# manikya7022/Continual-Learning-for-Dynamic-Video-Quality-Enhancement

Measured on AMD Instinct MI355X. Metric: train frames/sec (2x SR, T=3, 540p->1080p), higher is better.
Workload: dtype bf16

## Files before the change

continual-learning-for-dynamic-video-quality-enhancement_amd/csrc/conv_common.h:

```cpp
#pragma once
#include "common.h"

namespace nvq {

constexpr int TH = 8;
constexpr int TW = 32;
constexpr int NVQ_SMALL_IMAGE_TILES = 32;
constexpr int WG_C = 32;
constexpr int WGRAD_MAX_WG = 512;
constexpr int WGRAD_MAX_SLABS = 1536;

static inline int choose_nt(int cout) { return cout <= 16 ? 16 : (cout <= 32 ? 32 : 64); }

#ifdef NVQ_DEBUG_TOOLS
void set_conv_debug_mode(int m);
#endif
void conv_occupancy_bf16(int* out);

typedef short s16x4 __attribute__((ext_vector_type(4)));
typedef unsigned u32x4 __attribute__((ext_vector_type(4)));

constexpr int KCB = 32;

__host__ __device__ constexpr int ws_stride_halfs(int taps, int NT) { return ((taps * 4 * NT * 8 + 2047) / 2048) * 2048; }
// ... 15 lines not shown
              float* wpack, hipStream_t s);
struct PackJobDev { const float* w; float* wp; int cout_w, cin_w, taps, transpose, cout_keep, NT, ncz, nkc; long total; };
constexpr int PACK_BATCH = 48;
struct PackJobTable { PackJobDev j[PACK_BATCH]; };
int pack_batch_bf16(const PackJobTable& t, int n, hipStream_t s);
PackJobDev pack_job_bf16(const nvq_pack_job& j);
int conv_forward_bf16(const nvq_conv_desc& d, int vec_ok, hipStream_t s);
int conv_wgrad_bf16(const nvq_wgrad_desc& d, int nsplit, int nci, int nco, int tilesX, int tilesY, int ntiles,
                    hipStream_t s);
int upsampler_tail_bf16(const nvq_conv_desc& d, const float* frames, int T, int t_center, int Cimg, int s, float* out,
                        unsigned char* pass, hipStream_t st);
int rdb_tail_bf16(const nvq_conv_desc& d3, const nvq_conv_desc& dl, int vec3, int vecl, hipStream_t s);
int conv_forward_m32(const nvq_conv_desc& d, int variant, int dbg, hipStream_t s);
void conv_occupancy_m32(int* out);
bool wgrad_m32_takes(const nvq_wgrad_desc& d);
int conv_wgrad_m32(const nvq_wgrad_desc& d, hipStream_t s);

__device__ __forceinline__ void wgrad_bias_partial(const nvq_wgrad_desc& d, float4 bsum, float* lds, int nco, int cic,
                                                   int coc) {
    if (cic != 0 || d.dbias == nullptr) return;
    __syncthreads();
    st4(lds + 4 * threadIdx.x, bsum);
    __syncthreads();
    if (threadIdx.x < 32) {
        const int q = threadIdx.x >> 2, e = threadIdx.x & 3;
        float s = 0.f;
        for (int k = 0; k < 32; ++k) s += lds[4 * (8 * k + q) + e];
        float* bp = d.workspace + (size_t)WGRAD_MAX_SLABS * 9 * WG_C * WG_C;
        bp[((size_t)blockIdx.x * nco + coc) * WG_C + threadIdx.x] = s;
    }
}
// ... 180 lines not shown
```

continual-learning-for-dynamic-video-quality-enhancement_amd/csrc/conv_igemm.hip:

```cpp
#include "conv_common.h"

namespace nvq {

constexpr int KC = 16;
constexpr int XS_LD = 20;

__device__ __forceinline__ float pack_f32_elem(const float* __restrict__ w, int cout_w, int cin_w, int taps, int transpose,
                                               int cout_keep, int NT, int nkc, long idx) {
    long t = idx;
    const int j = t & 3; t >>= 2;
    const int n = t % NT; t /= NT;
    const int g = t & 3; t >>= 2;
    const int tap = t % taps; t /= taps;
    const int kc = t % nkc; t /= nkc;
    const int cz = (int)t;
    const int co = cz * NT + n;
    const int ch = kc * KC + 4 * g + j;
    float v = 0.f;
    if (!transpose) {
        if (co < cout_w && ch < cin_w) v = w[((long)co * cin_w + ch) * taps + tap];
    } else {
        if (co < cout_keep && ch < cout_w) v = w[((long)ch * cin_w + co) * taps + (taps - 1 - tap)];
    }
    return v;
// ... 676 lines not shown
            else if (gs == 2) NVQ_LAUNCH_CONV(2, KS, 2);             \
            else NVQ_LAUNCH_CONV(1, KS, 4);                          \
        }                                                            \
    } while (0)
    if (d.ksize == 3) NVQ_LAUNCH_CONV_KS(3);
    else NVQ_LAUNCH_CONV_KS(1);
#undef NVQ_LAUNCH_CONV_KS
#undef NVQ_LAUNCH_CONV
    return check_launch("conv_forward");
}

size_t nvq_wgrad_workspace_bytes(void) {
    return (size_t)WGRAD_MAX_SLABS * 9 * WG_C * WG_C * sizeof(float) + (size_t)512 * 256 * sizeof(float);
}

static int wgrad_partial(const nvq_wgrad_desc* dp, nvq_wgrad_reduce_job* job, void* stream) {
    const nvq_wgrad_desc d = *dp;
    NVQ_REQUIRE(d.math == NVQ_MATH_F32 || d.math == NVQ_MATH_BF16, "conv_wgrad: math mode %d", d.math);
    NVQ_REQUIRE(d.ksize == 1 || d.ksize == 3, "conv_wgrad: ksize %d", d.ksize);
    NVQ_REQUIRE(d.cin % 4 == 0 && d.x_ld % 4 == 0 && d.x_coff % 4 == 0 && aligned16(d.x),
                "conv_wgrad: x must be 16-byte addressable");
    NVQ_REQUIRE(d.dy_ld % 4 == 0 && d.dy_coff % 4 == 0 && aligned16(d.dy),
                "conv_wgrad: dy must be 16-byte addressable");
    NVQ_REQUIRE(d.cin_w > 0 && d.cin_w <= d.cin && d.cout > 0, "conv_wgrad: channels");
    NVQ_REQUIRE(!(d.x_bf16 | d.dy_bf16) || d.math == NVQ_MATH_BF16, "conv_wgrad: bf16 tensors need NVQ_MATH_BF16");
    NVQ_REQUIRE(!d.x_bf16 || (d.cin % 8 == 0 && d.x_ld % 8 == 0 && d.x_coff % 8 == 0), "conv_wgrad: bf16 x alignment");
    NVQ_REQUIRE(!d.dy_bf16 || (d.cout % 8 == 0 && d.dy_ld % 8 == 0 && d.dy_coff % 8 == 0), "conv_wgrad: bf16 dy alignment");
    NVQ_REQUIRE(d.math != NVQ_MATH_BF16 || d.dy_coff + ((d.cout + 3) & ~3) <= d.dy_ld,
                "conv_wgrad(bf16): the dy slice must be readable up to a multiple of 4 channels");
    NVQ_REQUIRE(d.workspace_bytes >= nvq_wgrad_workspace_bytes(), "conv_wgrad: workspace too small");
    NVQ_REQUIRE(!d.x_plane || (d.math == NVQ_MATH_BF16 && d.x_bf16 && d.x_coff == 0 && d.cin % 32 == 0 &&
                               (d.x_ld == 32 || d.x_ld == 64 || d.x_ld == 128) && d.x_ld <= d.cin &&
                               (size_t)d.x_plane == (size_t)d.n * d.h * d.w * 32),
                "conv_wgrad: a slice-planar x needs NVQ_MATH_BF16, bf16 storage, cin %% 32 == 0, x_coff 0, x_ld in {32, 64, 128} "
                "and x_plane = n*h*w*32");
    const int taps = d.ksize * d.ksize;
    const int nci = (d.cin_w + WG_C - 1) / WG_C, nco = (d.cout + WG_C - 1) / WG_C;
    const int tilesX = (d.w + TW - 1) / TW, tilesY = (d.h + TH - 1) / TH;
    const int ntiles = tilesX * tilesY * d.n;
    int nsplit = WGRAD_MAX_WG / (nci * nco);
    if (nsplit < 1) nsplit = 1;
    if (nsplit > ntiles) nsplit = ntiles;
    if (nsplit >= 8) nsplit &= ~7;
    NVQ_REQUIRE((size_t)nsplit * nci * nco * taps * WG_C * WG_C * sizeof(float) <= d.workspace_bytes,
                "conv_wgrad: %d x %d channel chunks exceed the workspace", nci, nco);
    hipStream_t s = (hipStream_t)stream;
    const dim3 grid(nsplit, nci, nco);
    int rc;
    if (d.math == NVQ_MATH_BF16) {
        const int used = conv_wgrad_bf16(d, nsplit, nci, nco, tilesX, tilesY, ntiles, s);
        if (used < 0) return used;
        rc = check_launch("conv_wgrad_bf16");
        if (used > 0) nsplit = used;
    } else {
        if (d.ksize == 3)
            hipLaunchKernelGGL((wgrad_f32_kernel<3>), grid, dim3(256), 0, s, d, tilesX, tilesY, ntiles, nci, nco);
        else
            hipLaunchKernelGGL((wgrad_f32_kernel<1>), grid, dim3(256), 0, s, d, tilesX, tilesY, ntiles, nci, nco);
        rc = check_launch("conv_wgrad");
    }
    if (rc) return rc;
    *job = nvq_wgrad_reduce_job{d.workspace, d.workspace + (size_t)WGRAD_MAX_SLABS * 9 * WG_C * WG_C, d.dw, d.dbias, nsplit, nci,
                                nco, taps, d.cout, d.cin_w, d.alpha, d.accumulate};
    return NVQ_OK;
}

int nvq_conv_wgrad(const nvq_wgrad_desc* dp, void* stream) {
    nvq_wgrad_reduce_job j;
    const int rc = wgrad_partial(dp, &j, stream);
    if (rc) return rc;
    return launch_wgrad_reduce_bias(j.part, j.nsplit, j.nci, j.nco, j.taps, j.cout, j.cin_w, j.alpha, j.accumulate, j.dw,
                                    j.bias_part, j.dbias, (hipStream_t)stream);
}

int nvq_conv_wgrad_partial(const nvq_wgrad_desc* dp, nvq_wgrad_reduce_job* job, void* stream) {
    NVQ_REQUIRE(job != nullptr, "conv_wgrad_partial: job");
    return wgrad_partial(dp, job, stream);
}

int nvq_wgrad_reduce_batch(const nvq_wgrad_reduce_job* jobs, int n, void* stream) {
    NVQ_REQUIRE(n >= 0 && (n == 0 || jobs != nullptr), "wgrad_reduce_batch: jobs");
    for (int i = 0; i < n; ++i)
        NVQ_REQUIRE(jobs[i].part && jobs[i].dw && jobs[i].nsplit > 0 && jobs[i].nci > 0 && jobs[i].nco > 0 &&
                        (jobs[i].taps == 1 || jobs[i].taps == 9) && (!jobs[i].dbias || jobs[i].bias_part),
                    "wgrad_reduce_batch: job %d is not one nvq_conv_wgrad_partial filled in", i);
    for (int i0 = 0; i0 < n; i0 += WR_MAX_JOBS) {
        const int m = n - i0 < WR_MAX_JOBS ? n - i0 : WR_MAX_JOBS;
        WgradReduceTable t;
        long need = 1;
        for (int i = 0; i < m; ++i) {
            t.j[i] = jobs[i0 + i];
            const long total = (long)t.j[i].nci * t.j[i].nco * t.j[i].taps * WG_C * WG_C;
// ... 21 lines not shown
```

continual-learning-for-dynamic-video-quality-enhancement_amd/csrc/wgrad_m32.hip:

```cpp
#include <type_traits>
#include "conv_common.h"

namespace nvq {

namespace {

typedef float f32x16 __attribute__((ext_vector_type(16)));
typedef s16x4 __attribute__((address_space(3))) * lds_s16x4_ptr;

constexpr int WM_TR = 4;
constexpr int WM_NTHR = 512;
constexpr int WM_HW = TW + 2, WM_HH = 2 + 2, WM_NPY = WM_HW * WM_HH;
constexpr int WM_YBYTES = WM_NPY * 64;
constexpr int WM_UPX = 2 * TW;
constexpr int WM_DYT = 384;

__device__ __forceinline__ void gload16(u32x4& dst, const void* p) {
    asm volatile("global_load_dwordx4 %0, %1, off" : "=&v"(dst) : "v"(p) : "memory");
}
__device__ __forceinline__ void gload16s(u32x4& dst, const void* sbase, unsigned voff) {
    asm volatile("global_load_dwordx4 %0, %1, %2" : "=&v"(dst) : "v"(voff), "s"(sbase) : "memory");
}
template <int N>
__device__ __forceinline__ void vm_wait() {
    asm volatile("s_waitcnt vmcnt(%0)" ::"n"(N) : "memory");
}
__device__ __forceinline__ void hold(u32x4& r) { asm volatile("" : "+v"(r)); }

template <int NCI>
struct WmCfg {
    static constexpr int CB = (NCI + 1) / 2;
    static constexpr int UBYTES = WM_UPX * NCI * 64;
    static constexpr int XPIECES = WM_UPX * NCI * 4;
    static constexpr int XPT = (XPIECES + WM_NTHR - 1) / WM_NTHR;
    static constexpr int LDS = 2 * UBYTES + 2 * WM_YBYTES;
};

// ... 240 lines not shown
#pragma unroll
            for (int e = 0; e < 8; ++e) scratch[8 * dt + e] = bsum[e];
        }
        __syncthreads();
        if (tid < 32) {
            const int piece = tid >> 3, e = tid & 7;
            float sum = 0.f;
            for (int k = piece; k < WM_DYT; k += 4) sum += scratch[8 * k + e];
            float* bp = d.workspace + (size_t)WGRAD_MAX_SLABS * 9 * WG_C * WG_C;
            bp[(size_t)blockIdx.x * WG_C + tid] = sum;
        }
    }
    (void)dyw;
}

template <int NCI, int NCO>
__global__ __launch_bounds__(WM_NTHR, 4) void wgrad1_m32_kernel(const nvq_wgrad_desc d, int tilesX, int tilesY, int ntiles) {
    constexpr int UBYTES = WM_UPX * NCI * 64, YB = WM_UPX * NCO * 64;
    constexpr int XPT = (WM_UPX * NCI * 4 + WM_NTHR - 1) / WM_NTHR;
    constexpr int YTHR = WM_UPX * NCO * 4;
    static_assert(NCI <= 8 && NCO <= 2 && 2 * (UBYTES + YB) <= 80 * 1024, "1x1 configuration");
    __shared__ __attribute__((aligned(1024))) unsigned char lds[2 * (UBYTES + YB)];
    constexpr int YOFF = 2 * UBYTES;

    const int tid = threadIdx.x;
    const int lane = tid & 63;
    const int wave = __builtin_amdgcn_readfirstlane(tid >> 6);
    const int H = d.h, W = d.w;
    const int G = gridDim.x;
    const int mytiles = ((int)blockIdx.x < ntiles) ? (ntiles - 1 - (int)blockIdx.x) / G + 1 : 0;
    const int U = 2 * mytiles;
    const __bf16* x16 = reinterpret_cast<const __bf16*>(d.x);
    const __bf16* dy16 = reinterpret_cast<const __bf16*>(d.dy);
    const int LU = d.x_plane ? d.x_ld >> 5 : NCI;

    const int xcol = (tid >> 2) & 31, xsub = tid & 3, xrow = (wave >> 1) & 1, xblk0 = wave >> 2;
    const unsigned v_lead = (unsigned)((xcol * d.x_ld + 8 * xsub) * 2), v_plane = (unsigned)((xcol * 32 + 8 * xsub) * 2);
    const int ypx = tid / (4 * NCO), yq = tid % (4 * NCO), yrow = NCO == 2 ? wave >> 2 : (wave >> 1) & 1, ycol = ypx & 31;
    const bool ythr = tid < YTHR;
    const unsigned v_y = (unsigned)((ycol * d.dy_ld + 8 * yq) * 2);
    struct Set { u32x4 x[XPT]; u32x4 y; bool xok, yok; };
    constexpr int S = XPT + 1;
    int c_n = 0, c_ty = 0, c_tx = 0, c_unit = 0;
    {
        int bt = xcd_tile((int)blockIdx.x, ntiles);
        c_tx = bt % tilesX; bt /= tilesX;
        c_ty = bt % tilesY;
        c_n = bt / tilesY;
    }
    const int c_step = G >> 3;
    auto load = [&](int u, Set& st) {
        if ((u >> 1) != (c_unit >> 1)) {
            if ((G & 7) == 0) {
                c_tx += c_step;
                while (c_tx >= tilesX) { c_tx -= tilesX; ++c_ty; }
                while (c_ty >= tilesY) { c_ty -= tilesY; ++c_n; }
            } else {
// ... 11 lines not shown
            st.xok = row_ok && xcol < W - x0;
            const unsigned vl = st.xok ? v_lead : 0u, vp = st.xok ? v_plane : 0u;
#pragma unroll
            for (int k = 0; k < XPT; ++k) {
                const int blk = xblk0 + 2 * k < NCI ? xblk0 + 2 * k : 0;
                if (blk < LU) gload16s(st.x[k], x16 + ((size_t)rel * (unsigned)d.x_ld + d.x_coff + 32u * blk), vl);
                else gload16s(st.x[k], x16 + ((size_t)blk * d.x_plane + rel * 32u), vp);
            }
        }
        {
            const bool row_ok = y0 + yrow < H;
            const size_t rel = (size_t)((c_n * H + (row_ok ? y0 + yrow : y0)) * W + x0);
            st.yok = ythr && row_ok && ycol < W - x0;
            gload16s(st.y, dy16 + (rel * d.dy_ld + d.dy_coff), st.yok ? v_y : 0u);
        }
    };
    float bsum[8];
#pragma unroll
    for (int e = 0; e < 8; ++e) bsum[e] = 0.f;
    auto write = [&](int u, Set& st) {
        const u32x4 z = {0u, 0u, 0u, 0u};
        unsigned char* slot = lds + (u & 1) * UBYTES + tid * 16;
#pragma unroll
        for (int k = 0; k < XPT; ++k) {
            hold(st.x[k]);
            if (xblk0 + 2 * k < NCI) *reinterpret_cast<u32x4*>(slot + k * (WM_NTHR * 16)) = st.xok ? st.x[k] : z;
        }
        hold(st.y);
        if (ythr) {
            const u32x4 v = st.yok ? st.y : z;
            *reinterpret_cast<u32x4*>(lds + YOFF + (u & 1) * YB + ((yq >> 2) * WM_UPX + ypx) * 64 + (yq & 3) * 16) = v;
            bsum[0] += bf_lo(v[0]); bsum[1] += bf_hi(v[0]); bsum[2] += bf_lo(v[1]); bsum[3] += bf_hi(v[1]);
            bsum[4] += bf_lo(v[2]); bsum[5] += bf_hi(v[2]); bsum[6] += bf_lo(v[3]); bsum[7] += bf_hi(v[3]);
        }
    };
    const int r = lane & 15, hb = (lane >> 4) & 1, h = lane >> 5;
    const int q = r >> 2, p = r & 3;
    const unsigned fbase = (unsigned)((8 * h + q) * 64 + hb * 32 + 8 * p);
    f32x16 acc[NCO];
#pragma unroll
    for (int a = 0; a < NCO; ++a)
#pragma unroll
        for (int e = 0; e < 16; ++e) acc[a][e] = 0.f;
    auto tr2 = [&](const unsigned char* a) -> bf16x8 {
        const s16x4 v0 = __builtin_amdgcn_ds_read_tr16_b64_v4i16((lds_s16x4_ptr)a);
        const s16x4 v1 = __builtin_amdgcn_ds_read_tr16_b64_v4i16((lds_s16x4_ptr)(a + 256));
        return __builtin_bit_cast(bf16x8, __builtin_shufflevector(v0, v1, 0, 1, 2, 3, 4, 5, 6, 7));
    };
    Set sa, sb;
    auto unit = [&](int u, Set& st) {
        asm volatile("s_waitcnt lgkmcnt(0)" ::: "memory");
        __builtin_amdgcn_s_barrier();
        if (wave < NCI) {
            const unsigned char* xs = lds + (u & 1) * UBYTES + wave * (WM_UPX * 64) + fbase;
            const unsigned char* ys = lds + YOFF + (u & 1) * YB + fbase;
            bf16x8 a[4], b[4][NCO];
#pragma unroll
            for (int k = 0; k < 4; ++k) {
                a[k] = tr2(xs + k * (16 * 64));
#pragma unroll
                for (int co = 0; co < NCO; ++co) b[k][co] = tr2(ys + co * (WM_UPX * 64) + k * (16 * 64));
            }
#pragma unroll
            for (int k = 0; k < 4; ++k)
#pragma unroll
                for (int co = 0; co < NCO; ++co) acc[co] = __builtin_amdgcn_mfma_f32_32x32x16_bf16(a[k], b[k][co], acc[co], 0, 0, 0);
        }
        if (u + 1 < U) {
            if (u + 2 < U) vm_wait<S>(); else vm_wait<0>();
            write(u + 1, st);
            if (u + 3 < U) load(u + 3, st);
        }
    };
    if (U > 0) {
        load(0, sa);
        load(1, sb);
        vm_wait<S>();
        write(0, sa);
        if (2 < U) load(2, sa);
    }
#pragma unroll 1
    for (int u = 0; u < U; u += 2) {
        unit(u, sb);
        unit(u + 1, sa);
    }
    if (wave < NCI) {
#pragma unroll
        for (int co = 0; co < NCO; ++co) {
            float* part = d.workspace + ((size_t)(blockIdx.x * NCI + wave) * NCO + co) * (WG_C * WG_C);
#pragma unroll
            for (int e = 0; e < 16; ++e) part[((e & 3) + 8 * (e >> 2) + 4 * h) * WG_C + (lane & 31)] = acc[co][e];
        }
// ... 16 lines not shown
    }
}

bool wgrad_m32_takes(const nvq_wgrad_desc& d) {
    if (!(d.x_bf16 && d.dy_bf16) || d.cin_w != d.cin || d.cin % 32 != 0 || d.cout % 32 != 0) return false;
    const int nci = d.cin / 32, nco = d.cout / 32;
    if ((size_t)(d.x_plane ? (size_t)nci * d.x_plane : (size_t)d.n * d.h * d.w * d.x_ld) >= ((size_t)1 << 32) ||
        (size_t)d.n * d.h * d.w * d.dy_ld >= ((size_t)1 << 31))
        return false;
    const long ntiles = (long)((d.w + TW - 1) / TW) * ((d.h + WM_TR - 1) / WM_TR) * d.n;
    if ((d.variant & 15) != 2 && ntiles < 4 * (d.ksize == 3 ? 256 : 512)) return false;
    if (d.ksize == 3) return d.x_plane && d.cout == 32 && nci >= 3 && nci <= 6 && d.cin >= d.x_ld;
    return nci >= 2 && nci <= 8 && nco <= 2 && (!d.x_plane || d.cin >= d.x_ld);
}

int conv_wgrad_m32(const nvq_wgrad_desc& d, hipStream_t s) {
    const int tilesX = (d.w + TW - 1) / TW, tilesY = (d.h + WM_TR - 1) / WM_TR;
    const int ntiles = tilesX * tilesY * d.n;
    const int nci = d.cin / 32, nco = d.cout / 32;
    int wgs = d.ksize == 3 ? 256 : 512;
    if (wgs > ntiles) wgs = ntiles;
    if (wgs >= 8) wgs &= ~7;
    NVQ_REQUIRE((size_t)wgs * nci * nco * d.ksize * d.ksize <= (size_t)WGRAD_MAX_SLABS * 9 && wgs <= 512,
                "conv_wgrad(bf16, all-ci): %d workgroups x %d x %d blocks exceed the workspace", wgs, nci, nco);
    if (d.ksize == 1) {
#define NVQ_LAUNCH_W1(NCI, NCO) \
    hipLaunchKernelGGL((wgrad1_m32_kernel<NCI, NCO>), dim3(wgs), dim3(WM_NTHR), 0, s, d, tilesX, tilesY, ntiles)
#define NVQ_W1_ROW(NCI) do { if (nco == 1) NVQ_LAUNCH_W1(NCI, 1); else NVQ_LAUNCH_W1(NCI, 2); } while (0)
        switch (nci) {
            case 2: NVQ_W1_ROW(2); break;
            case 3: NVQ_W1_ROW(3); break;
            case 4: NVQ_W1_ROW(4); break;
            case 5: NVQ_W1_ROW(5); break;
            case 6: NVQ_W1_ROW(6); break;
            case 7: NVQ_W1_ROW(7); break;
            default: NVQ_W1_ROW(8); break;
        }
#undef NVQ_W1_ROW
#undef NVQ_LAUNCH_W1
        return wgs;
    }
#define NVQ_LAUNCH_WM(NCI) hipLaunchKernelGGL((wgrad_m32_kernel<NCI>), dim3(wgs), dim3(WM_NTHR), 0, s, d, tilesX, tilesY, ntiles)
    switch (nci) {
// ... 12 lines not shown
```

continual-learning-for-dynamic-video-quality-enhancement_amd/nerve_cl/_engine.py:

```python
from __future__ import annotations

import os
from typing import Dict, Optional

import torch

from . import _nvq as K
from ._nvq import Sl

GROWTH = 32
LAYERS = 5
CORR_LD = 96
BN_EPS = 1e-5
BN_MOM = 0.1

_ws_cache: Dict[torch.device, torch.Tensor] = {}

DEBUG_CAPTURE: Optional[dict] = None

_TAIL_ROWS = int(os.environ.get("NVQ_TAIL_ROWS", "0"))


def _fused_tail_ok(math: int, x: torch.Tensor, Cimg: int, scale: int) -> bool:
    return (math == K.MATH_BF16 and x.dtype == torch.bfloat16 and scale in (2, 3, 4)
# ... 378 lines not shown
            return None
        self.writes[name] = self.writes.get(name, 0) + 1
        return self.G[name]

    def sink(self, name: str) -> torch.Tensor:
        g = self.get(name)
        return g if g is not None else torch.empty_like(self.P[name])

    def check(self) -> None:
        bad = {n: c for n, c in self.writes.items() if c != 1}
        missing = self.plan.wgrad - set(self.writes)
        assert not bad and not missing, f"backward plan: gradients written {bad}, never written {sorted(missing)}"


def _wgrad(x: Sl, cin_w: int, dy: Sl, G: _Grads, wname: str, bname: Optional[str], ws, ksize,
           alpha=1.0, math=K.MATH_F32):
    dw, db = G.get(wname), G.get(bname) if bname else None
    if dw is None and db is None:
        return
    if dw is None:
        dw = torch.empty_like(G.P[wname])
    if isinstance(ws, _ReduceQueue):
        K.conv_wgrad(x, cin_w, dy, dw, db, ws.ws(), ksize, alpha=alpha, math=math, defer=ws.jobs)
    else:
        K.conv_wgrad(x, cin_w, dy, dw, db, ws, ksize, alpha=alpha, math=math)


def extract_features(P: Dict[str, torch.Tensor], frames: torch.Tensor, F: int, math: int = K.MATH_F32,
                     act_dtype: torch.dtype = torch.float32) -> torch.Tensor:
    B, Tv, _, H, W = frames.shape
    out = _new(frames.device, Tv, B, H, W, F)
    for t0 in range(0, Tv, K.MAX_T):
        n = min(K.MAX_T, Tv - t0)
        part = frames[:, t0:t0 + n].contiguous()
        _extract(P, part, list(range(n)), F, False, math, act_dtype, Sl(out[t0:t0 + n].view(n * B, H, W, F)), n * B, None,
                 Saved())
    return out


def backward(P: Dict[str, torch.Tensor], sv: Saved, dout: torch.Tensor, G: Dict[str, torch.Tensor],
# ... 72 lines not shown
    K.conv_forward(Sl(dg), packs.get("gff.0.weight", True, F, F), None, gout, 3, math=math)
    _capture("dfused", (lambda: dfeat_c16.float()) if feat16 else dfeat_c)
    _capture("dres", lambda: gout.t[..., :F].float())

    K.TIMER_TAG = "rdb"
    ctr = F if (math == K.MATH_BF16 and F % 32 == 0) else 0
    reqs = []
    for k in range(nb):
        pre = f"residual_blocks.{k}."
        if f"rdb.{k}" not in run:
            continue
        wb, wbx = K.rdb_backward_weights(P[pre + "lff.weight"], [P[pre + f"layers.{i}.0.weight"] for i in range(LAYERS)], F)
        reqs += [(wb[j], False, F + GROWTH * j, None) for j in range(LAYERS)] + [(wbx, False, g.CAT, None)]
    mirror = K.conv_pack_many(reqs, math)
    ran = [k for k in range(nb) if f"rdb.{k}" in run]
    for k in range(nb - 1, -1, -1):
        if k not in ran:
            break
        cat = sv.cats[k]
        dcat = dcats[k & 1]
        pre = f"residual_blocks.{k}."
        gout = dcat.x()
        _wgrad(cat.inp(g.CAT), g.CAT, gout, G, pre + "lff.weight", pre + "lff.bias", wq, 1, alpha=0.2, math=math)
        j = ran.index(k)
        wpb = mirror[j * (LAYERS + 1):(j + 1) * (LAYERS + 1)]
        lowest = 0 if f"rdb.{k}" in dxs else min(
            [i for i in range(LAYERS) if pre + f"layers.{i}.0.weight" in G.plan.wgrad or pre + f"layers.{i}.0.bias" in G.plan.wgrad],
            default=LAYERS)
        for i in range(LAYERS - 1, lowest - 1, -1):
            cinb = F + GROWTH * (LAYERS - 1 - i)
            dy = dcat.y(LAYERS - 1 - i)
            if sv.bits is not None:
                K.conv_forward(dcat.inp(cinb), wpb[LAYERS - 1 - i], None, dy, 3,
                               math=math, bits=sv.bits[k][i], bits_mode=2, center_cin=ctr)
            else:
                K.conv_forward(dcat.inp(cinb), wpb[LAYERS - 1 - i], None, dy, 3,
                               mask=cat.y(i), mask_c0=0, mask_c1=GROWTH, math=math, center_cin=ctr)
            cin = F + GROWTH * i
            _wgrad(cat.inp(cin), cin, dy, G, pre + f"layers.{i}.0.weight", pre + f"layers.{i}.0.bias", wq, 3,
                   math=math)
        if f"rdb.{k}" not in dxs:
            break
        nxt = dcats[(k - 1) & 1].x() if k > 0 else Sl(dagg)
        K.conv_forward(dcat.inp(g.CAT), wpb[LAYERS], None, nxt, 3, res=gout, math=math, center_cin=ctr)
    K.TIMER_TAG = ""
    if "cbam" not in run:
        return None
# ... 333 lines not shown
```

continual-learning-for-dynamic-video-quality-enhancement_amd/nerve_cl/_nvq.py:

```python
from __future__ import annotations

import ctypes as C
import os
from typing import Dict, Optional, Sequence

import torch

_HERE = os.path.dirname(os.path.abspath(__file__))
LIB_PATH = os.environ.get("NVQ_LIB", os.path.join(os.path.dirname(_HERE), "libnvq.so"))

MATH_F32 = 0
MATH_BF16 = 1
MAX_T = 8

_lib = None

vp, ci, cl, cf, sz = C.c_void_p, C.c_int, C.c_long, C.c_float, C.c_size_t


class ConvDesc(C.Structure):
    _fields_ = [
        ("inp", vp), ("in_ld", ci), ("in_coff", ci), ("cin", ci),
        ("wpack", vp),
        ("bias", vp),
# ... 62 lines not shown

SIGNATURES = {
    "nvq_version": (ci, []),
    "nvq_last_error": (C.c_char_p, []),
    "nvq_conv_pack_floats": (sz, [ci, ci, ci, ci]),
    "nvq_conv_pack": (ci, [vp, ci, ci, ci, ci, ci, ci, ci, vp, vp]),
    "nvq_conv_forward": (ci, [C.POINTER(ConvDesc), vp]),
    "nvq_rdb_tail_forward": (ci, [C.POINTER(ConvDesc), C.POINTER(ConvDesc), vp]),
    "nvq_rdb_backward_weights_floats": (sz, [ci]),
    "nvq_rdb_backward_weights": (ci, [vp, vp, vp, vp, vp, vp, ci, vp, vp]),
    "nvq_sizeof_conv_desc": (sz, []),
    "nvq_wgrad_workspace_bytes": (sz, []),
    "nvq_conv_wgrad": (ci, [C.POINTER(WgradDesc), vp]),
    "nvq_conv_wgrad_partial": (ci, [C.POINTER(WgradDesc), C.POINTER(WgradReduceJob), vp]),
    "nvq_wgrad_reduce_batch": (ci, [C.POINTER(WgradReduceJob), ci, vp]),
    "nvq_sizeof_wgrad_desc": (sz, []),
    "nvq_sizeof_wgrad_reduce_job": (sz, []),
    "nvq_conv_pack_batch": (ci, [vp, ci, ci, vp]),
    "nvq_head_forward": (ci, [vp, ci, ci, ci, ci, ci, _IP, ci, vp, vp, ci, vp, ci, ci, vp, ci, vp]),
    "nvq_head_wgrad": (ci, [vp, ci, ci, ci, ci, ci, _IP, ci, vp, ci, vp, ci, vp, ci, ci, vp, vp, vp, sz, ci, ci, vp]),
    "nvq_dwconv_forward": (ci, [vp, ci, vp, ci, vp, ci, ci, ci, ci, ci, ci, ci, vp, vp, vp]),
    "nvq_dwconv_wgrad": (ci, [vp, ci, vp, ci, ci, ci, ci, ci, vp, vp, sz, ci, ci, ci, vp, vp]),
    "nvq_bn_stats": (ci, [vp, ci, ci, ci, ci, ci, ci, cf, cf, _IP, vp, vp, vp, vp, vp, sz, ci, vp]),
    "nvq_bn_eval_stats": (ci, [vp, vp, ci, ci, cf, vp, vp, vp]),
    "nvq_bn_apply_relu": (ci, [vp, ci, ci, ci, ci, ci, ci, vp, vp, vp, vp, vp, ci, vp, ci, ci, ci, vp, ci, ci, ci, ci, ci, vp]),
    "nvq_bn_relu_backward": (ci, [vp, ci, vp, ci, ci, ci, ci, ci, ci, vp, vp, vp, vp, ci, vp, ci, vp, vp, vp, sz, ci, ci, ci, ci, vp]),
    "nvq_dwconv_backward": (ci, [vp, ci, vp, vp, ci, vp, vp, ci, vp, ci, ci, ci, vp, vp, vp, vp, vp, sz, vp]),
    "nvq_dwconv_backward_ex": (ci, [vp, ci, vp, vp, ci, vp, vp, ci, vp, ci, ci, ci, vp, vp, vp, vp, vp, sz, ci, vp]),
    "nvq_dwpw_forward": (ci, [vp, ci, vp, vp, vp, vp, ci, vp, ci, ci, ci, ci, ci, ci, cf, cf, _IP, vp, vp, vp, vp, vp, sz, vp]),
    "nvq_pw_bn_backward": (ci, [vp, ci, ci, vp, ci, vp, ci, ci, ci, ci, ci, vp, vp, vp, vp, ci, vp, vp, ci, vp, vp, vp, vp, vp, sz, vp]),
# ... 449 lines not shown
    d.alpha, d.accumulate, d.math = alpha, int(accumulate), math
    d.x_bf16, d.dy_bf16, d.x_plane = x.bf16, dy.bf16, x.plane
    d.variant = variant
    if defer is not None:
        job = WgradReduceJob()
        check(lib().nvq_conv_wgrad_partial(C.byref(d), C.byref(job), stream()), "nvq_conv_wgrad_partial")
        defer.append((job, (ws, dw, dbias)))
        return
    check(lib().nvq_conv_wgrad(C.byref(d), stream()), "nvq_conv_wgrad")
    if ev0 is not None:
        TIMER.stop(ev0, f"wgrad_{'bf16' if math == MATH_BF16 else 'f32'}_kernel<{ksize}>", 2.0 * n * h * w * cin_w * dy.c * ksize * ksize,
                   n * h * w * (cin_w * (2.0 if x.bf16 else 4.0) + dy.c * (2.0 if dy.bf16 else 4.0)),
                   f"n{n} cin{cin_w}{'h' if x.bf16 else ''} cout{dy.c}{'h' if dy.bf16 else ''}")


def wgrad_reduce_batch(jobs: list) -> None:
    if not jobs:
        return
    arr = (WgradReduceJob * len(jobs))(*[j for j, _ in jobs])
    check(lib().nvq_wgrad_reduce_batch(arr, len(jobs), stream()), "nvq_wgrad_reduce_batch")
    jobs.clear()


def _nhwc4(src: Sl):
    n, h, w, _ = src.t.shape
    return n, src.c, h, w


def gather_nchw(jobs: "Sequence[tuple[Sl, torch.Tensor]]") -> None:
    if not jobs:
# ... 667 lines not shown
```

include/nvq.h:

```cpp
#ifndef NVQ_H
#define NVQ_H

#include <stddef.h>
#include <stdint.h>

#ifdef __cplusplus
extern "C" {
#endif

#define NVQ_OK 0
#define NVQ_EINVAL (-1)
#define NVQ_ELAUNCH (-2)
#define NVQ_EWORKSPACE (-3)

#define NVQ_MATH_F32 0
#define NVQ_MATH_BF16 1

#define NVQ_MAX_T 8

int nvq_version(void);
const char* nvq_last_error(void);


size_t nvq_conv_pack_floats(int cout, int cin_store, int ksize, int math);
// ... 44 lines not shown
    float* workspace; size_t workspace_bytes;
    int n, h, w, ksize;
    float alpha; int accumulate; int math;
    int x_bf16, dy_bf16;
    unsigned x_plane;
    int variant;
} nvq_wgrad_desc;
size_t nvq_wgrad_workspace_bytes(void);
int nvq_conv_wgrad(const nvq_wgrad_desc* d, void* stream);
typedef struct {
    const float* part; const float* bias_part; float* dw; float* dbias;
    int nsplit, nci, nco, taps, cout, cin_w; float alpha; int accumulate;
} nvq_wgrad_reduce_job;
int nvq_conv_wgrad_partial(const nvq_wgrad_desc* d, nvq_wgrad_reduce_job* job, void* stream);
int nvq_wgrad_reduce_batch(const nvq_wgrad_reduce_job* jobs, int n, void* stream);
size_t nvq_sizeof_wgrad_desc(void);
size_t nvq_sizeof_wgrad_reduce_job(void);

int nvq_pw_bn_backward(const float* dy, int dy_ld, int dy_bf16, const float* p, int p_ld, const float* d, int d_ld,
                       int N, int group_images, int H, int W, const float* mean, const float* invstd,
                       const float* gamma, const float* beta, int training, const float* weight, float* dd, int dd_ld,
                       float* dgamma, float* dbeta, float* dweight, const float* sums_in, float* workspace,
                       size_t workspace_bytes, void* stream);
#define NVQ_NO_WGRAD 2
int nvq_pw_bn_backward_ex(const float* dy, int dy_ld, int dy_bf16, const float* p, int p_ld, const float* d, int d_ld,
                          int N, int group_images, int H, int W, const float* mean, const float* invstd,
                          const float* gamma, const float* beta, int training, const float* weight, float* dd, int dd_ld,
                          float* dgamma, float* dbeta, float* dweight, const float* sums_in, float* workspace,
                          size_t workspace_bytes, int flags, void* stream);

// ... 348 lines not shown
```

Baseline: 78.47.

## Fuse LFF 1x1 weight-gradient with last RDB layer input-gradient in one kernel

Adds a DG variant of the 1x1 all-ci wgrad kernel in which an otherwise idle wave also computes the input gradient of the last dense layer. It reads the dy tile already staged in LDS, multiplies it by the centre tap of the packed 3x3 weights, applies the ReLU bit mask and writes the bf16 result. The separate masked conv_forward dgrad launch for that layer is skipped whenever the fused path is taken, saving a kernel launch and a second read of dy. In exchange the kernel uses more LDS, adds an extra per-pixel mask load to the pipeline and splits the MFMA groups, which may lower occupancy or throughput of the wgrad kernel.

```diff
diff --git a/continual-learning-for-dynamic-video-quality-enhancement_amd/csrc/conv_common.h b/continual-learning-for-dynamic-video-quality-enhancement_amd/csrc/conv_common.h
--- a/continual-learning-for-dynamic-video-quality-enhancement_amd/csrc/conv_common.h
+++ b/continual-learning-for-dynamic-video-quality-enhancement_amd/csrc/conv_common.h
@@ -53,7 +53,9 @@
 int conv_forward_m32(const nvq_conv_desc& d, int variant, int dbg, hipStream_t s);
 void conv_occupancy_m32(int* out);
 bool wgrad_m32_takes(const nvq_wgrad_desc& d);
-int conv_wgrad_m32(const nvq_wgrad_desc& d, hipStream_t s);
+struct LffDgrad { const __bf16* wc; const unsigned* bits; __bf16* out; int out_ld, out_coff; };
+bool lff_dgrad_takes(const nvq_wgrad_desc& d, const LffDgrad& f);
+int conv_wgrad_m32(const nvq_wgrad_desc& d, hipStream_t s, const LffDgrad* f = nullptr);
 
 __device__ __forceinline__ void wgrad_bias_partial(const nvq_wgrad_desc& d, float4 bsum, float* lds, int nco, int cic,
                                                    int coc) {
diff --git a/continual-learning-for-dynamic-video-quality-enhancement_amd/csrc/conv_igemm.hip b/continual-learning-for-dynamic-video-quality-enhancement_amd/csrc/conv_igemm.hip
--- a/continual-learning-for-dynamic-video-quality-enhancement_amd/csrc/conv_igemm.hip
+++ b/continual-learning-for-dynamic-video-quality-enhancement_amd/csrc/conv_igemm.hip
@@ -714,7 +714,7 @@
     return (size_t)WGRAD_MAX_SLABS * 9 * WG_C * WG_C * sizeof(float) + (size_t)512 * 256 * sizeof(float);
 }
 
-static int wgrad_partial(const nvq_wgrad_desc* dp, nvq_wgrad_reduce_job* job, void* stream) {
+static int wgrad_partial(const nvq_wgrad_desc* dp, nvq_wgrad_reduce_job* job, void* stream, const LffDgrad* fuse = nullptr) {
     const nvq_wgrad_desc d = *dp;
     NVQ_REQUIRE(d.math == NVQ_MATH_F32 || d.math == NVQ_MATH_BF16, "conv_wgrad: math mode %d", d.math);
     NVQ_REQUIRE(d.ksize == 1 || d.ksize == 3, "conv_wgrad: ksize %d", d.ksize);
@@ -734,6 +734,7 @@
                                (size_t)d.x_plane == (size_t)d.n * d.h * d.w * 32),
                 "conv_wgrad: a slice-planar x needs NVQ_MATH_BF16, bf16 storage, cin %% 32 == 0, x_coff 0, x_ld in {32, 64, 128} "
                 "and x_plane = n*h*w*32");
+    if (fuse != nullptr && !lff_dgrad_takes(d, *fuse)) return NVQ_NOT_TAKEN;
     const int taps = d.ksize * d.ksize;
     const int nci = (d.cin_w + WG_C - 1) / WG_C, nco = (d.cout + WG_C - 1) / WG_C;
     const int tilesX = (d.w + TW - 1) / TW, tilesY = (d.h + TH - 1) / TH;
@@ -748,7 +749,7 @@
     const dim3 grid(nsplit, nci, nco);
     int rc;
     if (d.math == NVQ_MATH_BF16) {
-        const int used = conv_wgrad_bf16(d, nsplit, nci, nco, tilesX, tilesY, ntiles, s);
+        const int used = fuse ? conv_wgrad_m32(d, s, fuse) : conv_wgrad_bf16(d, nsplit, nci, nco, tilesX, tilesY, ntiles, s);
         if (used < 0) return used;
         rc = check_launch("conv_wgrad_bf16");
         if (used > 0) nsplit = used;
@@ -776,6 +777,23 @@
 int nvq_conv_wgrad_partial(const nvq_wgrad_desc* dp, nvq_wgrad_reduce_job* job, void* stream) {
     NVQ_REQUIRE(job != nullptr, "conv_wgrad_partial: job");
     return wgrad_partial(dp, job, stream);
+}
+
+int nvq_lff_wgrad_dgrad_partial(const nvq_wgrad_desc* dp, const float* wpack, const unsigned* bits, float* out, int out_ld,
+                                int out_coff, nvq_wgrad_reduce_job* job, void* stream) {
+    NVQ_REQUIRE(job != nullptr, "lff_wgrad_dgrad_partial: job");
+    const LffDgrad f{reinterpret_cast<const __bf16*>(wpack), bits, reinterpret_cast<__bf16*>(out), out_ld, out_coff};
+    return wgrad_partial(dp, job, stream, &f);
+}
+
+int nvq_lff_wgrad_dgrad(const nvq_wgrad_desc* dp, const float* wpack, const unsigned* bits, float* out, int out_ld, int out_coff,
+                        void* stream) {
+    nvq_wgrad_reduce_job j;
+    const LffDgrad f{reinterpret_cast<const __bf16*>(wpack), bits, reinterpret_cast<__bf16*>(out), out_ld, out_coff};
+    const int rc = wgrad_partial(dp, &j, stream, &f);
+    if (rc) return rc;
+    return launch_wgrad_reduce_bias(j.part, j.nsplit, j.nci, j.nco, j.taps, j.cout, j.cin_w, j.alpha, j.accumulate, j.dw,
+                                    j.bias_part, j.dbias, (hipStream_t)stream);
 }
 
 int nvq_wgrad_reduce_batch(const nvq_wgrad_reduce_job* jobs, int n, void* stream) {
diff --git a/continual-learning-for-dynamic-video-quality-enhancement_amd/csrc/wgrad_m32.hip b/continual-learning-for-dynamic-video-quality-enhancement_amd/csrc/wgrad_m32.hip
--- a/continual-learning-for-dynamic-video-quality-enhancement_amd/csrc/wgrad_m32.hip
+++ b/continual-learning-for-dynamic-video-quality-enhancement_amd/csrc/wgrad_m32.hip
@@ -21,6 +21,10 @@
 __device__ __forceinline__ void gload16s(u32x4& dst, const void* sbase, unsigned voff) {
     asm volatile("global_load_dwordx4 %0, %1, %2" : "=&v"(dst) : "v"(voff), "s"(sbase) : "memory");
 }
+__device__ __forceinline__ void gload4s(unsigned& dst, const void* sbase, unsigned voff) {
+    asm volatile("global_load_dword %0, %1, %2" : "=&v"(dst) : "v"(voff), "s"(sbase) : "memory");
+}
+__device__ __forceinline__ void hold(unsigned& r) { asm volatile("" : "+v"(r)); }
 template <int N>
 __device__ __forceinline__ void vm_wait() {
     asm volatile("s_waitcnt vmcnt(%0)" ::"n"(N) : "memory");
@@ -291,13 +295,17 @@
     (void)dyw;
 }
 
-template <int NCI, int NCO>
-__global__ __launch_bounds__(WM_NTHR, 4) void wgrad1_m32_kernel(const nvq_wgrad_desc d, int tilesX, int tilesY, int ntiles) {
+template <int NCI, int NCO, bool DG>
+__global__ __launch_bounds__(WM_NTHR, 4) void wgrad1_m32_kernel(const nvq_wgrad_desc d, int tilesX, int tilesY, int ntiles,
+                                                                const LffDgrad f) {
     constexpr int UBYTES = WM_UPX * NCI * 64, YB = WM_UPX * NCO * 64;
+    constexpr int WOFF = 2 * (UBYTES + YB), WCB = 2 * 4 * 32 * 16;
+    constexpr int MOFF = WOFF + WCB;
+    static_assert(!DG || (NCO == 2 && NCI <= 7), "the input gradient needs 64 dy channels and a wave without an input block");
     constexpr int XPT = (WM_UPX * NCI * 4 + WM_NTHR - 1) / WM_NTHR;
     constexpr int YTHR = WM_UPX * NCO * 4;
-    static_assert(NCI <= 8 && NCO <= 2 && 2 * (UBYTES + YB) <= 80 * 1024, "1x1 configuration");
-    __shared__ __attribute__((aligned(1024))) unsigned char lds[2 * (UBYTES + YB)];
+    static_assert(NCI <= 8 && NCO <= 2 && 2 * (UBYTES + YB) + (DG ? WCB + 512 : 0) <= 80 * 1024, "1x1 configuration");
+    __shared__ __attribute__((aligned(1024))) unsigned char lds[2 * (UBYTES + YB) + (DG ? WCB + 512 : 0)];
     constexpr int YOFF = 2 * UBYTES;
 
     const int tid = threadIdx.x;
@@ -316,8 +324,10 @@
     const int ypx = tid / (4 * NCO), yq = tid % (4 * NCO), yrow = NCO == 2 ? wave >> 2 : (wave >> 1) & 1, ycol = ypx & 31;
     const bool ythr = tid < YTHR;
     const unsigned v_y = (unsigned)((ycol * d.dy_ld + 8 * yq) * 2);
-    struct Set { u32x4 x[XPT]; u32x4 y; bool xok, yok; };
+    struct Set { u32x4 x[XPT]; u32x4 y; unsigned m; bool xok, yok; };
     constexpr int S = XPT + 1;
+    const bool dgw = DG && wave == NCI;
+    const int mrow = lane >> 5, mcol = lane & 31;
     int c_n = 0, c_ty = 0, c_tx = 0, c_unit = 0;
     {
         int bt = xcd_tile((int)blockIdx.x, ntiles);
@@ -359,6 +369,12 @@
             st.yok = ythr && row_ok && ycol < W - x0;
             gload16s(st.y, dy16 + (rel * d.dy_ld + d.dy_coff), st.yok ? v_y : 0u);
         }
+        if constexpr (DG) {
+            if (dgw) {
+                const bool ok = y0 + mrow < H && x0 + mcol < W;
+                gload4s(st.m, f.bits + (size_t)c_n * H * W, ok ? (unsigned)(((y0 + mrow) * W + x0 + mcol) * 4) : 0u);
+            }
+        }
     };
     float bsum[8];
 #pragma unroll
@@ -378,6 +394,15 @@
             bsum[0] += bf_lo(v[0]); bsum[1] += bf_hi(v[0]); bsum[2] += bf_lo(v[1]); bsum[3] += bf_hi(v[1]);
             bsum[4] += bf_lo(v[2]); bsum[5] += bf_hi(v[2]); bsum[6] += bf_lo(v[3]); bsum[7] += bf_hi(v[3]);
         }
+        if constexpr (DG) {
+            if (dgw) {
+                hold(st.m);
+                reinterpret_cast<unsigned*>(lds + MOFF)[(u & 1) * WM_UPX + lane] = st.m;
+            }
+        }
+    };
+    auto wait_set = [&]() {
+        if (dgw) vm_wait<S + 1>(); else vm_wait<S>();
     };
     const int r = lane & 15, hb = (lane >> 4) & 1, h = lane >> 5;
     const int q = r >> 2, p = r & 3;
@@ -392,35 +417,117 @@
         const s16x4 v1 = __builtin_amdgcn_ds_read_tr16_b64_v4i16((lds_s16x4_ptr)(a + 256));
         return __builtin_bit_cast(bf16x8, __builtin_shufflevector(v0, v1, 0, 1, 2, 3, 4, 5, 6, 7));
     };
+    int o_n = c_n, o_ty = c_ty, o_tx = c_tx, o_unit = 0;
+    auto dgrad = [&](int u) {
+        if ((u >> 1) != (o_unit >> 1)) {
+            if ((G & 7) == 0) {
+                o_tx += c_step;
+                while (o_tx >= tilesX) { o_tx -= tilesX; ++o_ty; }
+                while (o_ty >= tilesY) { o_ty -= tilesY; ++o_n; }
+            } else {
+                int bt = xcd_tile((int)blockIdx.x + (u >> 1) * G, ntiles);
+                o_tx = bt % tilesX; bt /= tilesX;
+                o_ty = bt % tilesY;
+                o_n = bt / tilesY;
+            }
+        }
+        o_unit = u;
+        const int px = lane & 31;
+        const unsigned char* wl = lds + WOFF + lane * 16;
+        const unsigned char* ys = lds + YOFF + (u & 1) * YB + px * 64 + h * 16;
+        const unsigned* ml = reinterpret_cast<const unsigned*>(lds + MOFF) + (u & 1) * WM_UPX + px;
+#pragma unroll
+        for (int rw = 0; rw < 2; ++rw)
+#pragma unroll
+            for (int e = 0; e < 16; ++e) acc[rw][e] = 0.f;
+#pragma unroll
+        for (int k = 0; k < 4; ++k) {
+            const bf16x8 a = *reinterpret_cast<const bf16x8*>(wl + k * (2 * 32 * 16));
+            bf16x8 b[2];
+#pragma unroll
+            for (int rw = 0; rw < 2; ++rw)
+                b[rw] = *reinterpret_cast<const bf16x8*>(ys + (k >> 1) * (WM_UPX * 64) + rw * (TW * 64) + (k & 1) * 32);
+            __builtin_amdgcn_sched_barrier(0);
+#pragma unroll
+            for (int rw = 0; rw < 2; ++rw) acc[rw] = __builtin_amdgcn_mfma_f32_32x32x16_bf16(a, b[rw], acc[rw], 0, 0, 0);
+            __builtin_amdgcn_sched_barrier(0);
+        }
+        const int y0 = o_ty * WM_TR + 2 * (u & 1), gx = o_tx * TW + px;
+        __bf16* out16 = f.out;
+#pragma unroll
+        for (int rw = 0; rw < 2; ++rw) {
+            __builtin_amdgcn_sched_barrier(0);
+            const unsigned mw = ml[rw * TW] >> (4 * h);
+            unsigned o[4][2];
+#pragma unroll
+            for (int j = 0; j < 4; ++j) {
+                float v[4];
+#pragma unroll
+                for (int e = 0; e < 4; ++e) v[e] = (mw >> (8 * j + e)) & 1u ? acc[rw][4 * j + e] : 0.f;
+                const uint2 t = __builtin_bit_cast(uint2, (bf16x4){(__bf16)v[0], (__bf16)v[1], (__bf16)v[2], (__bf16)v[3]});
+                o[j][0] = t.x; o[j][1] = t.y;
+            }
+#pragma unroll
+            for (int p = 0; p < 2; ++p)
+#pragma unroll
+                for (int w2 = 0; w2 < 2; ++w2) {
+                    const auto sw = __builtin_amdgcn_permlane32_swap(o[2 * p][w2], o[2 * p + 1][w2], false, false);
+                    o[2 * p][w2] = sw[0]; o[2 * p + 1][w2] = sw[1];
+                }
+            const int gy = y0 + rw;
+            if (gy < H && gx < W) {
+                __bf16* op = out16 + ((size_t)(o_n * H + gy) * W + gx) * f.out_ld + f.out_coff + 8 * h;
+#pragma unroll
+                for (int p = 0; p < 2; ++p)
+                    *reinterpret_cast<u32x4*>(op + 16 * p) = (u32x4){o[2 * p][0], o[2 * p][1], o[2 * p + 1][0], o[2 * p + 1][1]};
+            }
+        }
+    };
     Set sa, sb;
     auto unit = [&](int u, Set& st) {
         asm volatile("s_waitcnt lgkmcnt(0)" ::: "memory");
         __builtin_amdgcn_s_barrier();
+        if constexpr (DG) {
+            if (dgw) dgrad(u);
+        }
         if (wave < NCI) {
             const unsigned char* xs = lds + (u & 1) * UBYTES + wave * (WM_UPX * 64) + fbase;
             const unsigned char* ys = lds + YOFF + (u & 1) * YB + fbase;
-            bf16x8 a[4], b[4][NCO];
-#pragma unroll
-            for (int k = 0; k < 4; ++k) {
-                a[k] = tr2(xs + k * (16 * 64));
-#pragma unroll
-                for (int co = 0; co < NCO; ++co) b[k][co] = tr2(ys + co * (WM_UPX * 64) + k * (16 * 64));
-            }
-#pragma unroll
-            for (int k = 0; k < 4; ++k)
-#pragma unroll
-                for (int co = 0; co < NCO; ++co) acc[co] = __builtin_amdgcn_mfma_f32_32x32x16_bf16(a[k], b[k][co], acc[co], 0, 0, 0);
+            constexpr int KG = DG ? 2 : 4;
+#pragma unroll
+            for (int k0 = 0; k0 < 4; k0 += KG) {
+                bf16x8 a[KG], b[KG][NCO];
+#pragma unroll
+                for (int k = 0; k < KG; ++k) {
+                    a[k] = tr2(xs + (k0 + k) * (16 * 64));
+#pragma unroll
+                    for (int co = 0; co < NCO; ++co) b[k][co] = tr2(ys + co * (WM_UPX * 64) + (k0 + k) * (16 * 64));
+                }
+                if constexpr (DG) __builtin_amdgcn_sched_barrier(0);
+#pragma unroll
+                for (int k = 0; k < KG; ++k)
+#pragma unroll
+                    for (int co = 0; co < NCO; ++co)
+                        acc[co] = __builtin_amdgcn_mfma_f32_32x32x16_bf16(a[k], b[k][co], acc[co], 0, 0, 0);
+                if constexpr (DG) __builtin_amdgcn_sched_barrier(0);
+            }
         }
         if (u + 1 < U) {
-            if (u + 2 < U) vm_wait<S>(); else vm_wait<0>();
+            if (u + 2 < U) wait_set(); else vm_wait<0>();
             write(u + 1, st);
             if (u + 3 < U) load(u + 3, st);
         }
     };
+    if constexpr (DG) {
+        constexpr int WS_HALFS = ws_stride_halfs(9, 32), CT = 4 * 4 * 32 * 8;
+        if (tid < WCB / 16)
+            *reinterpret_cast<u32x4*>(lds + WOFF + tid * 16) =
+                *reinterpret_cast<const u32x4*>(f.wc + (tid >> 7) * WS_HALFS + CT + (tid & 127) * 8);
+    }
     if (U > 0) {
         load(0, sa);
         load(1, sb);
-        vm_wait<S>();
+        wait_set();
         write(0, sa);
         if (2 < U) load(2, sa);
     }
@@ -467,7 +574,14 @@
     return nci >= 2 && nci <= 8 && nco <= 2 && (!d.x_plane || d.cin >= d.x_ld);
 }
 
-int conv_wgrad_m32(const nvq_wgrad_desc& d, hipStream_t s) {
+bool lff_dgrad_takes(const nvq_wgrad_desc& d, const LffDgrad& f) {
+    if (d.ksize != 1 || d.math != NVQ_MATH_BF16 || (d.variant & 15) == 1 || !wgrad_m32_takes(d)) return false;
+    return d.cout == 64 && d.cin / 32 <= 7 && d.x_plane != 0 && f.wc != nullptr && f.bits != nullptr && f.out != nullptr &&
+           f.out_ld >= 32 && f.out_ld % 8 == 0 && f.out_coff >= 0 && f.out_coff % 8 == 0 && f.out_coff + 32 <= f.out_ld &&
+           aligned16(f.out) && aligned16(f.wc);
+}
+
+int conv_wgrad_m32(const nvq_wgrad_desc& d, hipStream_t s, const LffDgrad* f) {
     const int tilesX = (d.w + TW - 1) / TW, tilesY = (d.h + WM_TR - 1) / WM_TR;
     const int ntiles = tilesX * tilesY * d.n;
     const int nci = d.cin / 32, nco = d.cout / 32;
@@ -477,9 +591,21 @@
     NVQ_REQUIRE((size_t)wgs * nci * nco * d.ksize * d.ksize <= (size_t)WGRAD_MAX_SLABS * 9 && wgs <= 512,
                 "conv_wgrad(bf16, all-ci): %d workgroups x %d x %d blocks exceed the workspace", wgs, nci, nco);
     if (d.ksize == 1) {
-#define NVQ_LAUNCH_W1(NCI, NCO) \
-    hipLaunchKernelGGL((wgrad1_m32_kernel<NCI, NCO>), dim3(wgs), dim3(WM_NTHR), 0, s, d, tilesX, tilesY, ntiles)
-#define NVQ_W1_ROW(NCI) do { if (nco == 1) NVQ_LAUNCH_W1(NCI, 1); else NVQ_LAUNCH_W1(NCI, 2); } while (0)
+#define NVQ_LAUNCH_W1(NCI, NCO, DG) \
+    hipLaunchKernelGGL((wgrad1_m32_kernel<NCI, NCO, DG>), dim3(wgs), dim3(WM_NTHR), 0, s, d, tilesX, tilesY, ntiles, \
+                       f ? *f : LffDgrad{})
+        if (f != nullptr) {
+            switch (nci) {
+                case 2: NVQ_LAUNCH_W1(2, 2, true); break;
+                case 3: NVQ_LAUNCH_W1(3, 2, true); break;
+                case 4: NVQ_LAUNCH_W1(4, 2, true); break;
+                case 5: NVQ_LAUNCH_W1(5, 2, true); break;
+                case 6: NVQ_LAUNCH_W1(6, 2, true); break;
+                default: NVQ_LAUNCH_W1(7, 2, true); break;
+            }
+            return wgs;
+        }
+#define NVQ_W1_ROW(NCI) do { if (nco == 1) NVQ_LAUNCH_W1(NCI, 1, false); else NVQ_LAUNCH_W1(NCI, 2, false); } while (0)
         switch (nci) {
             case 2: NVQ_W1_ROW(2); break;
             case 3: NVQ_W1_ROW(3); break;
diff --git a/continual-learning-for-dynamic-video-quality-enhancement_amd/nerve_cl/_engine.py b/continual-learning-for-dynamic-video-quality-enhancement_amd/nerve_cl/_engine.py
--- a/continual-learning-for-dynamic-video-quality-enhancement_amd/nerve_cl/_engine.py
+++ b/continual-learning-for-dynamic-video-quality-enhancement_amd/nerve_cl/_engine.py
@@ -416,16 +416,18 @@
 
 
 def _wgrad(x: Sl, cin_w: int, dy: Sl, G: _Grads, wname: str, bname: Optional[str], ws, ksize,
-           alpha=1.0, math=K.MATH_F32):
+           alpha=1.0, math=K.MATH_F32, dgrad=None) -> bool:
     dw, db = G.get(wname), G.get(bname) if bname else None
     if dw is None and db is None:
-        return
+        return False
     if dw is None:
         dw = torch.empty_like(G.P[wname])
-    if isinstance(ws, _ReduceQueue):
-        K.conv_wgrad(x, cin_w, dy, dw, db, ws.ws(), ksize, alpha=alpha, math=math, defer=ws.jobs)
-    else:
-        K.conv_wgrad(x, cin_w, dy, dw, db, ws, ksize, alpha=alpha, math=math)
+    queue = isinstance(ws, _ReduceQueue)
+    wsp, defer = (ws.ws(), ws.jobs) if queue else (ws, None)
+    if dgrad is not None and K.lff_wgrad_dgrad(x, cin_w, dy, dw, db, wsp, *dgrad, alpha=alpha, defer=defer):
+        return True
+    K.conv_wgrad(x, cin_w, dy, dw, db, wsp, ksize, alpha=alpha, math=math, defer=defer)
+    return False
 
 
 def extract_features(P: Dict[str, torch.Tensor], frames: torch.Tensor, F: int, math: int = K.MATH_F32,
@@ -528,6 +530,7 @@
         reqs += [(wb[j], False, F + GROWTH * j, None) for j in range(LAYERS)] + [(wbx, False, g.CAT, None)]
     mirror = K.conv_pack_many(reqs, math)
     ran = [k for k in range(nb) if f"rdb.{k}" in run]
+    fuse_lff = os.environ.get("NVQ_FUSE_LFF_BWD", "1") != "0"
     for k in range(nb - 1, -1, -1):
         if k not in ran:
             break
@@ -535,16 +538,21 @@
         dcat = dcats[k & 1]
         pre = f"residual_blocks.{k}."
         gout = dcat.x()
-        _wgrad(cat.inp(g.CAT), g.CAT, gout, G, pre + "lff.weight", pre + "lff.bias", wq, 1, alpha=0.2, math=math)
         j = ran.index(k)
         wpb = mirror[j * (LAYERS + 1):(j + 1) * (LAYERS + 1)]
         lowest = 0 if f"rdb.{k}" in dxs else min(
             [i for i in range(LAYERS) if pre + f"layers.{i}.0.weight" in G.plan.wgrad or pre + f"layers.{i}.0.bias" in G.plan.wgrad],
             default=LAYERS)
+        fuse4 = (fuse_lff and lowest <= LAYERS - 1 and sv.bits is not None and math == K.MATH_BF16 and ctr == F
+                 and sv.planar and pre + "lff.weight" in G.plan.wgrad)
+        have4 = _wgrad(cat.inp(g.CAT), g.CAT, gout, G, pre + "lff.weight", pre + "lff.bias", wq, 1, alpha=0.2, math=math,
+                       dgrad=(wpb[0], sv.bits[k][LAYERS - 1], dcat.y(0)) if fuse4 else None)
         for i in range(LAYERS - 1, lowest - 1, -1):
             cinb = F + GROWTH * (LAYERS - 1 - i)
             dy = dcat.y(LAYERS - 1 - i)
-            if sv.bits is not None:
+            if i == LAYERS - 1 and have4:
+                pass
+            elif sv.bits is not None:
                 K.conv_forward(dcat.inp(cinb), wpb[LAYERS - 1 - i], None, dy, 3,
                                math=math, bits=sv.bits[k][i], bits_mode=2, center_cin=ctr)
             else:
diff --git a/continual-learning-for-dynamic-video-quality-enhancement_amd/nerve_cl/_nvq.py b/continual-learning-for-dynamic-video-quality-enhancement_amd/nerve_cl/_nvq.py
--- a/continual-learning-for-dynamic-video-quality-enhancement_amd/nerve_cl/_nvq.py
+++ b/continual-learning-for-dynamic-video-quality-enhancement_amd/nerve_cl/_nvq.py
@@ -100,6 +100,8 @@
     "nvq_conv_wgrad": (ci, [C.POINTER(WgradDesc), vp]),
     "nvq_conv_wgrad_partial": (ci, [C.POINTER(WgradDesc), C.POINTER(WgradReduceJob), vp]),
     "nvq_wgrad_reduce_batch": (ci, [C.POINTER(WgradReduceJob), ci, vp]),
+    "nvq_lff_wgrad_dgrad": (ci, [C.POINTER(WgradDesc), vp, vp, vp, ci, ci, vp]),
+    "nvq_lff_wgrad_dgrad_partial": (ci, [C.POINTER(WgradDesc), vp, vp, vp, ci, ci, C.POINTER(WgradReduceJob), vp]),
     "nvq_sizeof_wgrad_desc": (sz, []),
     "nvq_sizeof_wgrad_reduce_job": (sz, []),
     "nvq_conv_pack_batch": (ci, [vp, ci, ci, vp]),
@@ -579,6 +581,46 @@
                    f"n{n} cin{cin_w}{'h' if x.bf16 else ''} cout{dy.c}{'h' if dy.bf16 else ''}")
 
 
+NOT_TAKEN = 1
+
+
+def lff_wgrad_dgrad(x: Sl, cin_w: int, dy: Sl, dw: torch.Tensor, dbias: Optional[torch.Tensor], ws: torch.Tensor,
+                    wpack: torch.Tensor, bits: torch.Tensor, out: Sl, *, alpha: float = 1.0, accumulate: bool = False,
+                    variant: int = 0, defer: Optional[list] = None) -> bool:
+    n, h, w, _ = x.t.shape
+    if not (out.bf16 and out.c == 32 and out.t.shape[:3] == x.t.shape[:3] and bits is not None and bits.dtype == torch.int32
+            and tuple(bits.shape) == (n, h, w) and bits.is_contiguous()):
+        return False
+    ev0 = TIMER.start() if TIMER is not None and defer is None else None
+    d = WgradDesc()
+    d.x, d.x_ld, d.x_coff, d.cin, d.cin_w = ptr(x.t), x.ld, x.coff, x.c, cin_w
+    d.dy, d.dy_ld, d.dy_coff, d.cout = ptr(dy.t), dy.ld, dy.coff, dy.c
+    d.dw, d.dbias = ptr(dw), ptr(dbias)
+    d.workspace, d.workspace_bytes = ptr(ws), ws.numel() * ws.element_size()
+    d.n, d.h, d.w, d.ksize = n, h, w, 1
+    d.alpha, d.accumulate, d.math = alpha, int(accumulate), MATH_BF16
+    d.x_bf16, d.dy_bf16, d.x_plane = x.bf16, dy.bf16, x.plane
+    d.variant = variant
+    if defer is not None:
+        job = WgradReduceJob()
+        rc = lib().nvq_lff_wgrad_dgrad_partial(C.byref(d), ptr(wpack), ptr(bits), ptr(out.t), out.ld, out.coff, C.byref(job),
+                                               stream())
+        if rc == NOT_TAKEN:
+            return False
+        check(rc, "nvq_lff_wgrad_dgrad_partial")
+        defer.append((job, (ws, dw, dbias)))
+        return True
+    rc = lib().nvq_lff_wgrad_dgrad(C.byref(d), ptr(wpack), ptr(bits), ptr(out.t), out.ld, out.coff, stream())
+    if rc == NOT_TAKEN:
+        return False
+    check(rc, "nvq_lff_wgrad_dgrad")
+    if ev0 is not None:
+        TIMER.stop(ev0, "wgrad_bf16_kernel<1>", 2.0 * n * h * w * (cin_w * dy.c + dy.c * out.c),
+                   n * h * w * (cin_w * 2.0 + dy.c * 2.0 + 4.0 + out.c * 2.0),
+                   f"n{n} cin{cin_w}h cout{dy.c}h +dgrad{out.c}h bitsR")
+    return True
+
+
 def wgrad_reduce_batch(jobs: list) -> None:
     if not jobs:
         return
diff --git a/include/nvq.h b/include/nvq.h
--- a/include/nvq.h
+++ b/include/nvq.h
@@ -82,6 +82,11 @@
 } nvq_wgrad_reduce_job;
 int nvq_conv_wgrad_partial(const nvq_wgrad_desc* d, nvq_wgrad_reduce_job* job, void* stream);
 int nvq_wgrad_reduce_batch(const nvq_wgrad_reduce_job* jobs, int n, void* stream);
+#define NVQ_NOT_TAKEN 1
+int nvq_lff_wgrad_dgrad(const nvq_wgrad_desc* d, const float* wpack, const unsigned* bits, float* out, int out_ld, int out_coff,
+                        void* stream);
+int nvq_lff_wgrad_dgrad_partial(const nvq_wgrad_desc* d, const float* wpack, const unsigned* bits, float* out, int out_ld,
+                                int out_coff, nvq_wgrad_reduce_job* job, void* stream);
 size_t nvq_sizeof_wgrad_desc(void);
 size_t nvq_sizeof_wgrad_reduce_job(void);
 
```

Measured after the change: 78.81 (median of 6 runs). No clear change (+0.4%).
